# annalam/seqkit

Hardware: AMD Instinct MI355X
Metric: M reads/s demultiplex (150bp, 96 barcodes) at 1/8 GPUs; % HBM roofline (higher is better)
Workload: dtype u8

## Files before the change

### seqkit_amd/csrc/sk_deflate.hip

```cpp
#include <hip/hip_runtime.h>

#include <algorithm>
#include <cstdlib>
#include <cstring>

#include "sk_internal.h"

namespace sk {

typedef uint32_t u32;
typedef unsigned long long u64;
typedef u32 u32x4 __attribute__((ext_vector_type(4)));

constexpr int kDefWaves = 4;
constexpr int kDefHashBits = 12;
constexpr u32 kDefMaxIn = 0xff00u;
constexpr int kNLL = 286, kND = 30;

struct DefLds {
	uint16_t head[1 << kDefHashBits];
	u32 freq[kNLL + kND];
	uint16_t code[kNLL + kND];
	uint8_t len[kNLL + kND + 2];
	u32 nfreq[2 * kNLL];
	uint16_t parent[2 * kNLL];
	uint16_t order[kNLL];
	uint8_t depth[2 * kNLL];
	u32 stage[128];
};

__device__ const uint8_t kPreLen[19] = {4, 5, 5, 5, 4, 4, 4, 4, 4, 4, 4, 4, 4, 4, 4, 4, 5, 5, 5};
__device__ const uint8_t kPreOrderD[19] = {16, 17, 18, 0, 8, 7, 9, 6, 10, 5, 11, 4, 12, 3, 13, 2, 14, 1, 15};

__device__ __forceinline__ void def_fence()
{
	__builtin_amdgcn_fence(__ATOMIC_RELEASE, "wavefront");
	__builtin_amdgcn_wave_barrier();
	__builtin_amdgcn_fence(__ATOMIC_ACQUIRE, "wavefront");
}
__device__ __forceinline__ u32 def_uniform(u32 v) { return (u32)__builtin_amdgcn_readfirstlane((int)v); }
__device__ __forceinline__ u32 def_rev(u32 code, u32 len) { return __builtin_bitreverse32(code) >> (32u - len); }

__device__ __forceinline__ u32 def_load4(const uint8_t *p)
{
	const uintptr_t a = (uintptr_t)p;
	const u32 *q = reinterpret_cast<const u32 *>(a & ~(uintptr_t)3);
	const u32 sh = (u32)(a & 3u);
	const u32 lo = q[0];
	return sh == 0u ? lo : __builtin_amdgcn_alignbyte(q[1], lo, sh);
}

__device__ __forceinline__ void def_len_code(u32 len, u32 &sym, u32 &xb, u32 &xv)
{
	const u32 l = len - 3u;
	if (l < 8u) { sym = 257u + l; xb = 0u; xv = 0u; return; }
	if (len == 258u) { sym = 285u; xb = 0u; xv = 0u; return; }
	const u32 nb = 31u - (u32)__builtin_clz(l);
	sym = 257u + 4u * (nb - 1u) + ((l >> (nb - 2u)) & 3u);
	xb = nb - 2u;
	xv = l & ((1u << xb) - 1u);
}
__device__ __forceinline__ void def_dist_code(u32 dist, u32 &sym, u32 &xb, u32 &xv)
{
	const u32 d = dist - 1u;
	if (d < 4u) { sym = d; xb = 0u; xv = 0u; return; }
	const u32 nb = 31u - (u32)__builtin_clz(d);
	sym = 2u * nb + ((d >> (nb - 1u)) & 1u);
	xb = nb - 1u;
	xv = d & ((1u << xb) - 1u);
}

__device__ __attribute__((noinline)) void def_huffman(int wave, int base, int n, int lane)
{
	extern __shared__ __attribute__((aligned(16))) uint8_t def_smem[];
	DefLds &L = reinterpret_cast<DefLds *>(def_smem)[def_uniform((u32)wave)];
	base = (int)def_uniform((u32)base); n = (int)def_uniform((u32)n);
	u32 *const freq = L.freq + base;
	for (int shift = 0;; shift++) {
		u32 used = 0u;
		for (int s0 = 0; s0 < n; s0 += 64) {
			const int s = s0 + lane;
			used += (u32)__popcll(__ballot(s < n && freq[s] != 0u));
		}
		for (int s = lane; s < n; s += 64) L.len[base + s] = 0;
		if (used == 0u) {
			if (lane == 0) { L.len[base] = 1; L.code[base] = 0; }
			def_fence();
			return;
		}
		if (used == 1u) {
			for (int s = lane; s < n; s += 64) if (freq[s] != 0u) { L.len[base + s] = 1; L.code[base + s] = 0; }
			def_fence();
			return;
		}
		for (int s = lane; s < n; s += 64) {
			const u32 f = freq[s];
			if (f == 0u) continue;
			const u32 fs = max(1u, f >> shift);
			u32 r = 0u;
			for (int t = 0; t < n; t++) {
				const u32 g = freq[t];
				if (g == 0u) continue;
				const u32 gs = max(1u, g >> shift);
				r += (gs < fs || (gs == fs && t < s)) ? 1u : 0u;
			}
			L.order[r] = (uint16_t)s;
			L.nfreq[r] = fs;
		}
		def_fence();
		{
			u32 li = 0u, ii = used, made = used;
			const u32 total = 2u * used - 1u;
			while (made < total) {
				u32 pick[2];
#pragma unroll
				for (int k = 0; k < 2; k++) {
					const bool leaf_ok = li < used, int_ok = ii < made;
					bool take_leaf = leaf_ok;
					if (leaf_ok && int_ok) take_leaf = def_uniform(L.nfreq[li]) <= def_uniform(L.nfreq[ii]);
					pick[k] = take_leaf ? li++ : ii++;
				}
				if (lane == 0) {
					L.nfreq[made] = L.nfreq[pick[0]] + L.nfreq[pick[1]];
					L.parent[pick[0]] = (uint16_t)made;
					L.parent[pick[1]] = (uint16_t)made;
				}
				def_fence();
				made++;
			}
			if (lane == 0) L.depth[total - 1u] = 0;
			def_fence();
			for (int i = (int)total - 2; i >= 0; i--) {
				if (lane == 0) L.depth[i] = (uint8_t)(L.depth[L.parent[i]] + 1);
				def_fence();
			}
		}
		u32 maxd = 0u;
		for (u32 r0 = 0; r0 < used; r0 += 64) {
			const u32 r = r0 + (u32)lane;
			u32 d = r < used ? L.depth[r] : 0u;
			for (int o = 32; o > 0; o >>= 1) d = max(d, (u32)__shfl_xor((int)d, o));
			maxd = max(maxd, d);
		}
		if (maxd > 15u) continue;
		for (u32 r = (u32)lane; r < used; r += 64u) L.len[base + L.order[r]] = L.depth[r];
		def_fence();
		break;
	}
	u32 cnt[16];
#pragma unroll
	for (int l = 0; l < 16; l++) cnt[l] = 0u;
	for (int s0 = 0; s0 < n; s0 += 64) {
		const int s = s0 + lane;
		const u32 ls = s < n ? L.len[base + s] : 0u;
#pragma unroll
		for (int l = 1; l < 16; l++) cnt[l] += (u32)__popcll(__ballot(ls == (u32)l));
	}
	u32 first[16];
	{
		u32 c = 0u;
		first[0] = 0u;
#pragma unroll
		for (int l = 1; l < 16; l++) { c = (c + cnt[l - 1]) << 1; first[l] = c; }
	}
	u32 run[16];
#pragma unroll
	for (int l = 0; l < 16; l++) run[l] = 0u;
	for (int s0 = 0; s0 < n; s0 += 64) {
		const int s = s0 + lane;
		const u32 ls = s < n ? L.len[base + s] : 0u;
#pragma unroll
		for (int l = 1; l < 16; l++) {
			const u64 m = __ballot(ls == (u32)l);
			if (ls == (u32)l) L.code[base + s] = (uint16_t)def_rev(first[l] + run[l] + __builtin_amdgcn_mbcnt_hi((u32)(m >> 32), __builtin_amdgcn_mbcnt_lo((u32)m, 0u)), (u32)l);
			run[l] += (u32)__popcll(m);
		}
	}
	def_fence();
}

struct DefBlock { u64 in_off; u32 in_len, pad; };
static_assert(sizeof(DefBlock) == 16, "== sk_deflate_block");

struct DefOut { u32 *dst; u32 words; u32 carry_bits; };

__global__ __launch_bounds__(kDefWaves * 64) void bgzf_deflate_kernel(const uint8_t *in, const DefBlock *blocks, int64_t n_blocks, uint8_t *out, u32 out_stride,
                                                                      u32 *tokens, u32 *result)
{
	extern __shared__ __attribute__((aligned(16))) uint8_t def_smem[];
	const int lane = threadIdx.x & 63;
	const int wave = __builtin_amdgcn_readfirstlane((int)(threadIdx.x >> 6));
	DefLds &L = reinterpret_cast<DefLds *>(def_smem)[wave];
	for (int64_t bi = (int64_t)blockIdx.x * kDefWaves + wave; bi < n_blocks; bi += (int64_t)gridDim.x * kDefWaves) {
		const u64 in_off = (u64)def_uniform((u32)blocks[bi].in_off) | ((u64)def_uniform((u32)(blocks[bi].in_off >> 32)) << 32);
		const u32 n = def_uniform(blocks[bi].in_len);
		const uint8_t *src = in + in_off;
		u32 *const tok = tokens + (size_t)bi * kDefMaxIn;
		u32 *const dst = reinterpret_cast<u32 *>(out + (size_t)bi * out_stride);
		for (int i = lane; i < (1 << kDefHashBits); i += 64) L.head[i] = 0;
		for (int i = lane; i < kNLL + kND; i += 64) L.freq[i] = 0u;
		def_fence();
		u32 ntok = 0u, skip = 0u;
		for (u32 c0 = 0; c0 < n; c0 += 64u) {
			const u32 p = c0 + (u32)lane;
			const u32 cnt = min(64u, n - c0);
			u32 mlen = 0u, mdist = 0u, v = 0u, h = 0u;
			const bool can = p + 4u <= n;
			if (can) {
				v = def_load4(src + p);
				h = (v * 2654435761u) >> (32 - kDefHashBits);
				const u32 cand1 = L.head[h];
				if (cand1 != 0u) {
					const u32 cand = cand1 - 1u;
					const u32 d = p - cand;
					if (d <= 32768u && def_load4(src + cand) == v) {
						u32 l = 4u;
						const u32 maxl = min(258u, n - p);
						while (l + 4u <= maxl) {
							const u32 x = def_load4(src + cand + l) ^ def_load4(src + p + l);
							if (x != 0u) { l += (u32)__builtin_ctz(x) >> 3; break; }
							l += 4u;
						}
						if (l + 4u > maxl) { while (l < maxl && src[cand + l] == src[p + l]) l++; }
						mlen = l; mdist = d;
					}
				}
			}
			def_fence();
			if (can) L.head[h] = (uint16_t)(p + 1u);
			u64 starts = 0ull;
			u32 q = skip;
			while (q < cnt) {
				const u32 l = (u32)__builtin_amdgcn_readlane((int)mlen, (int)q);
				starts |= 1ull << q;
				q += l >= 3u ? l : 1u;
			}
			skip = q - cnt;
			const bool mine = (starts >> lane) & 1ull;
			const bool is_match = mine && mlen >= 3u;
			if (mine) {
				const u32 rank = __builtin_amdgcn_mbcnt_hi((u32)(starts >> 32), __builtin_amdgcn_mbcnt_lo((u32)starts, 0u));
				u32 t;
				if (is_match) {
					t = 0x80000000u | ((mlen - 3u) << 16) | (mdist - 1u);
					u32 sym, xb, xv;
					def_len_code(mlen, sym, xb, xv);
					atomicAdd(&L.freq[sym], 1u);
					def_dist_code(mdist, sym, xb, xv);
					atomicAdd(&L.freq[kNLL + sym], 1u);
				} else {
					const u32 b = can ? (v & 0xffu) : (u32)src[p];
					t = b;
					atomicAdd(&L.freq[b], 1u);
				}
				tok[ntok + rank] = t;
			}
			ntok += (u32)__popcll(starts);
		}
		if (lane == 0) atomicAdd(&L.freq[256], 1u);
		def_fence();
		def_huffman(wave, 0, kNLL, lane);
		def_huffman(wave, kNLL, kND, lane);
		for (int i = lane; i < 128; i += 64) L.stage[i] = 0u;
		def_fence();
		u32 words = 0u, carry = 0u;
		auto put = [&](u64 bv, u32 nb) {
			u32 off = nb;
#pragma unroll
			for (int o = 1; o < 64; o <<= 1) {
				const u32 t = (u32)__shfl_up((int)off, o);
				if (lane >= o) off += t;
			}
			const u32 total = (u32)__builtin_amdgcn_readlane((int)off, 63);
			const u32 at = carry + off - nb;
			if (nb != 0u) {
				const u32 w = at >> 5, sh = at & 31u;
				const u64 lo = bv << sh;
				atomicOr(&L.stage[w], (u32)lo);
				if (sh + nb > 32u) atomicOr(&L.stage[w + 1u], (u32)(lo >> 32));
				if (sh + nb > 64u) atomicOr(&L.stage[w + 2u], (u32)(bv >> (64u - sh)));
			}
			def_fence();
			const u32 bits = carry + total;
			const u32 full = bits >> 5;
			u32 keep = 0u;
			if ((u32)lane < full) dst[words + (u32)lane] = L.stage[lane];
			if ((u32)lane + 64u < full) dst[words + 64u + (u32)lane] = L.stage[64 + lane];
			keep = def_uniform(L.stage[full]);
			def_fence();
			for (int i = lane; i < 128; i += 64) L.stage[i] = 0u;
			def_fence();
			if (lane == 0) L.stage[0] = keep;
			def_fence();
			words += full;
			carry = bits & 31u;
		};
		{
			u64 bv = 0ull;
			u32 nb = 0u;
			if (lane == 0) { bv = 1ull | (2ull << 1) | (29ull << 3) | (29ull << 8) | (15ull << 13); nb = 17u; }
			else if (lane <= 19) { bv = kPreLen[kPreOrderD[lane - 1]]; nb = 3u; }
			put(bv, nb);
		}
		{
			auto pre_code = [&](u32 s, u32 &cl) -> u32 {
				cl = kPreLen[s];
				u32 before = 0u;
				for (u32 t = 0; t < s; t++) before += kPreLen[t] == cl ? 1u : 0u;
				const u32 c = cl == 4u ? before : (13u << 1) + before;
				return def_rev(c, cl);
			};
			for (int s0 = 0; s0 < kNLL + kND; s0 += 64) {
				const int s = s0 + lane;
				u64 bv = 0ull;
				u32 nb = 0u;
				if (s < kNLL + kND) { u32 cl; bv = pre_code(L.len[s], cl); nb = cl; }
				put(bv, nb);
			}
		}
		for (u32 t0 = 0; t0 < ntok + 1u; t0 += 64u) {
			const u32 ti = t0 + (u32)lane;
			u64 bv = 0ull;
			u32 nb = 0u;
			if (ti < ntok) {
				const u32 t = tok[ti];
				if (t & 0x80000000u) {
					const u32 len = ((t >> 16) & 0xffu) + 3u, dist = (t & 0x7fffu) + 1u;
					u32 sym, xb, xv;
					def_len_code(len, sym, xb, xv);
					bv = L.code[sym]; nb = L.len[sym];
					bv |= (u64)xv << nb; nb += xb;
					def_dist_code(dist, sym, xb, xv);
					bv |= (u64)L.code[kNLL + sym] << nb; nb += L.len[kNLL + sym];
					bv |= (u64)xv << nb; nb += xb;
				} else {
					bv = L.code[t]; nb = L.len[t];
				}
			} else if (ti == ntok) {
				bv = L.code[256]; nb = L.len[256];
			}
			put(bv, nb);
		}
		if (carry != 0u) {
			if (lane == 0) dst[words] = L.stage[0];
			words++;
		}
		if (lane == 0) {
			const u32 nbytes = (words - (carry != 0u ? 1u : 0u)) * 4u + ((carry + 7u) >> 3);
			result[2 * bi] = nbytes;
			result[2 * bi + 1] = ntok;
		}
		def_fence();
	}
}

__device__ __forceinline__ u32 dcrc_mul(u32 a, u32 b)
{
	u32 r = 0u;
	for (int i = 0; i < 32; i++) {
		if (a & 0x80000000u) r ^= b;
		a <<= 1;
		b = (b >> 1) ^ ((b & 1u) ? 0xEDB88320u : 0u);
	}
	return r;
}
__global__ __launch_bounds__(256) void bgzf_crc_out_kernel(const uint8_t *in, const DefBlock *blocks, int64_t n_blocks, u32 *crc_out)
{
	__shared__ u32 tab[4][256];
	__shared__ u32 pw[20];
	{
		u32 c = threadIdx.x;
		for (int k = 0; k < 8; k++) c = (c >> 1) ^ ((c & 1u) ? 0xEDB88320u : 0u);
		tab[0][threadIdx.x] = c;
		__syncthreads();
		u32 t = c;
		for (int k = 1; k < 4; k++) { t = (t >> 8) ^ tab[0][t & 0xffu]; tab[k][threadIdx.x] = t; }
		if (threadIdx.x == 0) {
			u32 p = 0x00800000u;
			for (int k = 0; k < 20; k++) { pw[k] = p; p = dcrc_mul(p, p); }
		}
	}
	__syncthreads();
	const int lane = threadIdx.x & 63, wave = threadIdx.x >> 6;
	for (int64_t bi = (int64_t)blockIdx.x * 4 + wave; bi < n_blocks; bi += (int64_t)gridDim.x * 4) {
		const u32 n = blocks[bi].in_len;
		const uint8_t *p = in + blocks[bi].in_off;
		const u32 mis = (u32)((16u - ((uintptr_t)p & 15u)) & 15u);
		const u32 headn = mis < n ? mis : n;
		const u32 body = n - headn;
		const u32 piece = (((body + 63u) >> 6) + 15u) & ~15u;
		const u32 lo = headn + min(body, piece * (u32)lane), hi = headn + min(body, piece * (u32)lane + piece);
		u32 c = lane == 0 ? 0xFFFFFFFFu : 0u;
		u32 len = hi - lo;
		if (lane == 0) {
			for (u32 i = 0; i < headn; i++) c = tab[0][(c ^ p[i]) & 0xffu] ^ (c >> 8);
			len += headn;
		}
		u32 i = lo;
		for (; i + 16u <= hi; i += 16u) {
			const u32x4 w = *reinterpret_cast<const u32x4 *>(p + i);
#pragma unroll
			for (int k = 0; k < 4; k++) {
				const u32 x = c ^ w[k];
				c = tab[3][x & 0xffu] ^ tab[2][(x >> 8) & 0xffu] ^ tab[1][(x >> 16) & 0xffu] ^ tab[0][x >> 24];
			}
		}
		for (; i < hi; i++) c = tab[0][(c ^ p[i]) & 0xffu] ^ (c >> 8);
		for (int o = 1; o < 64; o <<= 1) {
			const u32 cr = __shfl_down(c, o), lr = __shfl_down(len, o);
			if ((lane & (2 * o - 1)) == 0 && lane + o < 64) {
				u32 sh = 0x80000000u;
				u32 nb = lr;
				for (int k = 0; nb != 0u; k++, nb >>= 1) if (nb & 1u) sh = dcrc_mul(sh, pw[k]);
				c = dcrc_mul(c, sh) ^ cr;
				len += lr;
			}
		}
		if (lane == 0) crc_out[bi] = c ^ 0xFFFFFFFFu;
	}
}

hipError_t launch_bgzf_deflate(const uint8_t *in, const void *blocks, int64_t n_blocks, uint8_t *out, uint32_t out_stride, uint32_t *tokens, uint32_t *result,
                               uint32_t *crc, int n_cu, hipStream_t st)
{
	if (n_blocks <= 0) return hipSuccess;
	static bool attr_set = false;
	const size_t lds = sizeof(DefLds) * kDefWaves;
	if (!attr_set) {
		hipError_t e = hipFuncSetAttribute(reinterpret_cast<const void *>(bgzf_deflate_kernel), hipFuncAttributeMaxDynamicSharedMemorySize, (int)lds);
		if (e != hipSuccess) return e;
		attr_set = true;
	}
	const int per_cu = std::max(1, (int)((160 * 1024) / lds));
	int64_t grid = (n_blocks + kDefWaves - 1) / kDefWaves;
	const int64_t cap = (int64_t)n_cu * per_cu * 4;
	if (grid > cap) grid = cap;
	bgzf_deflate_kernel<<<dim3((unsigned)grid), dim3(kDefWaves * 64), lds, st>>>(in, reinterpret_cast<const DefBlock *>(blocks), n_blocks, out, out_stride, tokens, result);
	hipError_t e = hipGetLastError();
	if (e != hipSuccess) return e;
	int64_t cgrid = (n_blocks + 3) / 4;
	if (cgrid > (int64_t)n_cu * 16) cgrid = (int64_t)n_cu * 16;
	bgzf_crc_out_kernel<<<dim3((unsigned)cgrid), dim3(256), 0, st>>>(in, reinterpret_cast<const DefBlock *>(blocks), n_blocks, crc);
	return hipGetLastError();
}

hipError_t launch_bgzf_crc(const uint8_t *in, const void *blocks, int64_t n_blocks, uint32_t *crc, int n_cu, hipStream_t st)
{
	if (n_blocks <= 0) return hipSuccess;
	int64_t cgrid = (n_blocks + 3) / 4;
	if (cgrid > (int64_t)n_cu * 16) cgrid = (int64_t)n_cu * 16;
	bgzf_crc_out_kernel<<<dim3((unsigned)cgrid), dim3(256), 0, st>>>(in, reinterpret_cast<const DefBlock *>(blocks), n_blocks, crc);
	return hipGetLastError();
}

size_t deflate_tokens_per_block() { return kDefMaxIn; }

}
```

### seqkit_amd/build.py

```python
from __future__ import annotations

import os
import shutil
import subprocess
import sys

ROOT = os.path.dirname(os.path.abspath(__file__))
REPO = os.path.dirname(ROOT)
CSRC = os.path.join(ROOT, "csrc")
LIBDIR = os.path.join(ROOT, "lib")
BINDIR = os.path.join(ROOT, "bin")
LIB_PATH = os.path.join(LIBDIR, "libseqkit_hip.so")

HIP_SOURCES = ["sk_kernels.hip", "sk_census.hip", "sk_inflate.hip", "sk_deflate.hip", "sk_bamtext.hip", "sk_bamwrite.hip", "sk_bamminimize.hip", "sk_bammarkdup.hip", "sk_bamsubsample.hip", "sk_bammerge.hip", "sk_bamcoverage.hip", "sk_bampair.hip", "sk_bamtarget.hip", "sk_capi.hip", "sk_bamfile.cpp", "sk_bamfile_reads.cpp", "sk_bamfile_out.cpp", "sk_bamfile_coverage.cpp", "sk_lut.cpp"]
HIP_DEPS = HIP_SOURCES + ["sk_internal.h", "sk_lut.h", "sk_bamblock.h", "sk_bamfmt.h", "sk_bamfile.h", "sk_passmem.h", "sk_hoststage.h", "sk_tileplan.h", "sk_censusplan.h", os.path.join(REPO, "include", "seqkit_hip.h")]
HIP_FLAGS = ["--offload-arch=gfx950", "-O3", "-std=c++17", "-fPIC", "-shared", "-Wall", "-Wno-unused-function"]


def library_inputs_digest() -> str:
    import hashlib
    h = hashlib.sha256()
    h.update(" ".join(HIP_FLAGS).encode())
    for d in HIP_DEPS:
        p = d if os.path.isabs(d) else os.path.join(CSRC, d)
        with open(p, "rb") as f:
            h.update(os.path.basename(p).encode() + b"\0" + f.read())
    return h.hexdigest()[:16]


def _hipcc() -> str:
    for cand in (os.environ.get("HIPCC"), shutil.which("hipcc"), "/opt/rocm/bin/hipcc"):
        if cand and os.path.exists(cand):
            return cand
    raise RuntimeError("hipcc not found: the gfx950 library cannot be built")


def _stale(target: str, deps: list[str]) -> bool:
    if not os.path.exists(target):
        return True
    t = os.path.getmtime(target)
    for d in deps:
        p = d if os.path.isabs(d) else os.path.join(CSRC, d)
        if os.path.exists(p) and os.path.getmtime(p) > t:
            return True
    return False


def _run(cmd: list[str], cwd: str) -> None:
    r = subprocess.run(cmd, cwd=cwd, stdout=subprocess.PIPE, stderr=subprocess.STDOUT, text=True)
    if r.returncode != 0:
        sys.stderr.write(r.stdout)
        raise RuntimeError("build failed: " + " ".join(cmd))


def build_library(force: bool = False, verbose: bool = False) -> str:
    os.makedirs(LIBDIR, exist_ok=True)
    if force or _stale(LIB_PATH, HIP_DEPS):
        cmd = [_hipcc()] + HIP_FLAGS + ["-o", LIB_PATH] + HIP_SOURCES + ["-ldl", "-lz", "-pthread"]
        if verbose:
            cmd.append("-Rpass-analysis=kernel-resource-usage")
        _run(cmd, CSRC)
    return LIB_PATH


def build_hosts(force: bool = False) -> list[str]:
    os.makedirs(BINDIR, exist_ok=True)
    out = []
    for name, srcs, libs in (("fasta", ["host_common.cpp", "host_inflate.cpp", "fasta_main.cpp", "fasta_text.cpp"], ["-lz", "-ldl"]),
                             ("sam", ["host_common.cpp", "host_inflate.cpp", "sam_main.cpp"], ["-lz", "-ldl"])):
        if not all(os.path.exists(os.path.join(CSRC, s)) for s in srcs):
            continue
        target = os.path.join(BINDIR, name)
        deps = srcs + ["host_common.h", "sam_pairing.h", "sk_bamfmt.h", os.path.join(REPO, "include", "seqkit_hip.h"), LIB_PATH]
        if force or _stale(target, deps):
            cmd = ["g++", "-O2", "-std=c++17", "-Wall", "-Wextra", "-pthread", "-I", os.path.join(REPO, "include"),
                   "-o", target] + srcs + ["-L", LIBDIR, "-lseqkit_hip", "-Wl,-rpath,$ORIGIN/../lib"] + libs
            _run(cmd, CSRC)
        out.append(target)
    return out


def build_all(force: bool = False) -> None:
    build_library(force=force)
    build_hosts(force=force)


if __name__ == "__main__":
    build_all(force="--force" in sys.argv)
    print(LIB_PATH)
```

### seqkit_amd/csrc/sk_bamfile.cpp

```cpp
#include <fcntl.h>
#include <hip/hip_runtime.h>
#include <sys/stat.h>
#include <unistd.h>
#include <zlib.h>

#include <algorithm>
#include <chrono>
#include <cstdio>
#include <cstdlib>
#include <condition_variable>
#include <cstring>
#include <memory>
#include <mutex>
#include <string>
#include <thread>
#include <vector>

#include "sk_bamfile.h"

using namespace bamfile;

namespace {

bool pread_full(int fd, uint8_t *dst, size_t n, uint64_t off)
{
	size_t got = 0;
	while (got < n) {
		const ssize_t r = pread(fd, dst + got, n - got, (off_t)(off + got));
		if (r < 0) { if (errno == EINTR) continue; return false; }
		if (r == 0) return false;
		got += (size_t)r;
	}
	return true;
}

}

struct Mapper {
	OutRange *r = nullptr;
	std::thread th;
	std::mutex m;
	std::condition_variable cv;
	size_t want = 0, have = 0;
	bool stop = false, failed = false;
	void start(OutRange *range)
	{
		r = range; have = r->mapped;
		th = std::thread([this] {
			(void)hipSetDevice(r->device);
			std::unique_lock<std::mutex> lk(m);
			for (;;) {
				cv.wait(lk, [this] { return stop || want > have; });
				if (stop) return;
				const size_t next = have + 1;
				lk.unlock();
				const bool ok = r->ensure(next);
				lk.lock();
				if (!ok) { failed = true; cv.notify_all(); return; }
				have = r->mapped;
				cv.notify_all();
			}
		});
	}
	void ask(size_t bytes) { std::lock_guard<std::mutex> lk(m); if (bytes > want) { want = std::min(bytes, r->reserved); cv.notify_all(); } }
	bool wait_for(size_t bytes) { std::unique_lock<std::mutex> lk(m); if (bytes > want) { want = std::min(bytes, r->reserved); cv.notify_all(); } cv.wait(lk, [&] { return failed || have >= bytes; }); return !failed; }
	~Mapper() { if (th.joinable()) { { std::lock_guard<std::mutex> lk(m); stop = true; cv.notify_all(); } th.join(); } }
};
struct Readers {
	int fd = -1;
	uint8_t *ring = nullptr;
	size_t chunk = 0;
	uint64_t fsize = 0, n_chunks = 0;
	int R = 0;
	std::vector<hipEvent_t> ev;
	std::vector<int64_t> ready, copied;
	std::vector<std::thread> th;
	std::mutex m;
	std::condition_variable cv;
	uint64_t next = 0;
	bool stop = false, failed = false;
	int device = 0;
	void start(int threads)
	{
		ready.assign((size_t)R, -1); copied.assign((size_t)R, -1);
		for (int t = 0; t < threads; t++) th.emplace_back([this] {
			(void)hipSetDevice(device);
			for (;;) {
				uint64_t k;
				{
					std::unique_lock<std::mutex> lk(m);
					if (stop || next >= n_chunks) return;
					k = next++;
					const int s = (int)(k % (uint64_t)R);
					if (k >= (uint64_t)R) {
						cv.wait(lk, [&] { return stop || copied[(size_t)s] == (int64_t)(k - (uint64_t)R); });
						if (stop) return;
					}
				}
				const int s = (int)(k % (uint64_t)R);
				if (k >= (uint64_t)R) (void)hipEventSynchronize(ev[(size_t)s]);
				const uint64_t off = k * chunk;
				const size_t len = (size_t)std::min<uint64_t>(chunk, fsize - off);
				const bool ok = pread_full(fd, ring + (size_t)s * chunk, len, off);
				std::lock_guard<std::mutex> lk(m);
				if (!ok) failed = true;
				ready[(size_t)s] = (int64_t)k;
				cv.notify_all();
			}
		});
	}
	bool wait_ready(uint64_t k)
	{
		std::unique_lock<std::mutex> lk(m);
		const int s = (int)(k % (uint64_t)R);
		cv.wait(lk, [&] { return failed || ready[(size_t)s] == (int64_t)k; });
		return !failed;
	}
	void done_with(uint64_t k)
	{
		std::lock_guard<std::mutex> lk(m);
		copied[(size_t)(k % (uint64_t)R)] = (int64_t)k;
		cv.notify_all();
	}
	~Readers()
	{
		{ std::lock_guard<std::mutex> lk(m); stop = true; cv.notify_all(); }
		for (auto &t : th) t.join();
	}
};

int bamfile::bam_file_front(sk_ctx *c, const char *path, Cleanup &cl, Front &fr, double info[8])
{
	const char *who = fr.who;
	Ranges *both = (Ranges *)sk::ctx_ext(c);
	if (!both) { both = new Ranges; sk::ctx_set_ext(c, both, Ranges::destroy); }
	if (both->reads.busy() || both->rw.busy() || both->pairs.busy()) {
		BF_HIP(hipStreamSynchronize(sk::ctx_stream(c)));
		BF_HIP(hipStreamSynchronize(sk::ctx_stream2(c)));
	}
	both->gen++;
	both->reads.stop();
	both->rw.stop();
	both->pairs.stop();
	cl.fd = open(path, O_RDONLY);
	if (cl.fd < 0) BF_LEAVE(1);
	struct stat sb;
	if (fstat(cl.fd, &sb) != 0 || !S_ISREG(sb.st_mode) || sb.st_size < 28) BF_LEAVE(2);
	const uint64_t fsize = (uint64_t)sb.st_size;
	const double t0 = now_ms();
	hipStream_t st = sk::ctx_stream(c), st2 = sk::ctx_stream2(c);
	cl.wait_for = {st, st2};

	int krc = SK_OK;
	uint64_t out_cap = std::max<uint64_t>(fsize * 6, (uint64_t)256 << 20);
	if (const char *ev = getenv("SK_BAMFILE_OUT_FACTOR")) { const int f = atoi(ev); if (f >= 1 && f <= 1100) out_cap = std::max<uint64_t>(fsize * (uint64_t)f, (uint64_t)1 << 20); }
	uint8_t *d_out = nullptr, *d_comp = nullptr;
	OutRange *range = nullptr, *crange = nullptr;
	if (!getenv("SK_BAMFILE_NO_VMM")) {
		int dev = 0;
		BF_HIP(hipGetDevice(&dev));
		if (both->out.va && both->out.reserved < out_cap + 256) both->out.release();
		if (both->comp.va && both->comp.reserved < fsize + 64) both->comp.release();
		const bool comp_mapped = fsize > ((uint64_t)8 << 30);
		if (!comp_mapped && both->comp.va) both->comp.release();
		if ((both->out.va || both->out.reserve(out_cap + 256, dev)) && (!comp_mapped || both->comp.va || both->comp.reserve(fsize + 64, dev))) {
			range = &both->out;
			crange = comp_mapped ? &both->comp : nullptr;
		}
	}
	Mapper mapper, cmapper;
	if (range) {
		out_cap = range->reserved - 256;
		d_out = range->va;
		if (crange) {
			d_comp = crange->va;
			cmapper.start(crange);
			cmapper.ask((size_t)fsize + 64);
		} else {
			d_comp = (uint8_t *)sk::ctx_keep(c, sk::kKeepComp, fsize + 64, false, &krc);
			if (!d_comp) return krc;
		}
		mapper.start(range);
		mapper.ask(std::min<size_t>((size_t)fsize * 2, range->reserved));
	} else if (sk::ctx_kept_bytes(c, sk::kKeepOut) >= out_cap + 64) {
		out_cap = sk::ctx_kept_bytes(c, sk::kKeepOut) - 64;
		d_out = (uint8_t *)sk::ctx_keep(c, sk::kKeepOut, out_cap + 64, false, &krc);
		d_comp = (uint8_t *)sk::ctx_keep(c, sk::kKeepComp, fsize + 64, false, &krc);
		if (!d_comp) return krc;
	} else {
		d_comp = (uint8_t *)sk::ctx_keep(c, sk::kKeepComp, fsize + 64, false, &krc);
		if (!d_comp) return krc;
		size_t free_b = 0, total_b = 0;
		BF_HIP(hipMemGetInfo(&free_b, &total_b));
		out_cap = std::min<uint64_t>(out_cap, (uint64_t)((free_b + sk::ctx_kept_bytes(c, sk::kKeepOut)) * 0.8));
		d_out = (uint8_t *)sk::ctx_keep(c, sk::kKeepOut, out_cap + 64, false, &krc);
		if (!d_out) BF_LEAVE(3);
	}

	size_t chunk = (size_t)4 << 20;
	if (const char *ev = getenv("SK_BAMFILE_CHUNK_LOG2")) { const int lg = atoi(ev); if (lg >= 12 && lg <= 30) chunk = (size_t)1 << lg; }
	int threads = 8;
	{ const unsigned hc = std::thread::hardware_concurrency(); if (hc >= 1 && hc < 8) threads = (int)hc; }
	if (const char *ev = getenv("SK_BAMFILE_THREADS")) { const int t = atoi(ev); if (t >= 1 && t <= 64) threads = t; }
	const int kBufs = threads + threads / 2 + 1;
	Readers rd;
	rd.fd = cl.fd; rd.chunk = chunk; rd.fsize = fsize; rd.R = kBufs;
	rd.ring = (uint8_t *)sk::ctx_keep(c, sk::kKeepPin, (size_t)kBufs * chunk, true, &krc);
	if (!rd.ring) return krc;
	BF_HIP(hipGetDevice(&rd.device));
	for (int i = 0; i < kBufs; i++) {
		hipEvent_t e;
		BF_HIP(hipEventCreateWithFlags(&e, hipEventDisableTiming));
		cl.events.push_back(e);
		rd.ev.push_back(e);
	}
	hipEvent_t ev_batch;
	BF_HIP(hipEventCreateWithFlags(&ev_batch, hipEventDisableTiming));
	cl.events.push_back(ev_batch);

	const size_t tab_cap = (size_t)(fsize / 8192) + 1024;
	struct BlockTable {
		sk_bgzf_block *p = nullptr;
		size_t n = 0;
		size_t size() const { return n; }
		sk_bgzf_block *data() const { return p; }
		sk_bgzf_block &operator[](size_t i) const { return p[i]; }
	} blocks;
	blocks.p = (sk_bgzf_block *)sk::ctx_keep(c, sk::kKeepTable, tab_cap * sizeof(sk_bgzf_block), true, &krc);
	if (!blocks.p) return krc;
	std::vector<uint64_t> bend;
	bend.reserve(tab_cap);
	sk_bgzf_block *d_blocks = (sk_bgzf_block *)sk::ctx_keep(c, sk::kKeepBlocks, tab_cap * sizeof(sk_bgzf_block), false, &krc);
	if (!d_blocks) return krc;
	uint32_t *d_status = (uint32_t *)sk::ctx_keep(c, sk::kKeepStatus, tab_cap * sizeof(uint32_t), false, &krc);
	if (!d_status) return krc;

	const double t_alloc = now_ms();
	const size_t slots = (size_t)sk::ctx_n_cu(c) * 16;
	size_t min_batch = 2 * slots;
	if (const char *ev = getenv("SK_BAMFILE_BATCH")) { const int v = atoi(ev); if (v >= 1) min_batch = (size_t)v; }
	bool whole_rounds = true, two_streams = true;
	if (const char *ev = getenv("SK_BAMFILE_ROUNDS")) whole_rounds = atoi(ev) != 0;
	if (const char *ev = getenv("SK_BAMFILE_STREAMS")) two_streams = atoi(ev) >= 2;
	hipStream_t st_b = st;
	hipEvent_t ev_b = nullptr;
	if (two_streams) {
		BF_HIP(hipStreamCreateWithFlags(&st_b, hipStreamNonBlocking));
		cl.streams.push_back(st_b);
		BF_HIP(hipEventCreateWithFlags(&ev_b, hipEventDisableTiming));
		cl.events.push_back(ev_b);
	}
	int n_batches = 0;
	uint64_t scan = 0, out_off = 0;
	size_t launched = 0;
	const uint64_t n_chunks = (fsize + chunk - 1) / chunk;
	uint8_t carry[65536 + 64];
	rd.n_chunks = n_chunks;
	rd.start(threads);
	for (uint64_t k = 0; k < n_chunks; k++) {
		const uint64_t c_off = k * chunk;
		const size_t c_len = (size_t)std::min<uint64_t>(chunk, fsize - c_off);
		uint8_t *buf = rd.ring + (size_t)(k % (uint64_t)kBufs) * chunk;
		if (!rd.wait_ready(k)) BF_LEAVE(4);
		if (crange && !cmapper.wait_for((size_t)(c_off + c_len) + 64)) BF_LEAVE(3);
		BF_HIP(hipMemcpyAsync(d_comp + c_off, buf, c_len, hipMemcpyHostToDevice, st2));
		BF_HIP(hipEventRecord(rd.ev[(size_t)(k % (uint64_t)kBufs)], st2));
		const uint64_t have = c_off + c_len;
		auto bytes = [&](uint64_t off, size_t n) -> const uint8_t * {
			if (off >= c_off) return buf + (off - c_off);
			if (n > sizeof carry || !pread_full(cl.fd, carry, n, off)) return nullptr;
			return carry;
		};
		while (scan + 18 <= have) {
			const uint8_t *h = bytes(scan, 18);
			if (!h) BF_LEAVE(5);
			if (h[0] != 31 || h[1] != 139 || h[2] != 8 || !(h[3] & 4)) BF_LEAVE(6);
			const size_t xlen = (size_t)h[10] | ((size_t)h[11] << 8);
			if (scan + 12 + xlen > have) break;
			const uint8_t *x = bytes(scan, 12 + xlen);
			if (!x) BF_LEAVE(7);
			size_t bsize = 0;
			for (size_t o = 12; o + 4 <= 12 + xlen;) {
				const size_t slen = (size_t)x[o + 2] | ((size_t)x[o + 3] << 8);
				if (x[o] == 'B' && x[o + 1] == 'C' && slen == 2 && o + 6 <= 12 + xlen) { bsize = ((size_t)x[o + 4] | ((size_t)x[o + 5] << 8)) + 1; break; }
				o += 4 + slen;
			}
			if (bsize == 0 || bsize < 12 + xlen + 8) BF_LEAVE(8);
			if (scan + bsize > have) break;
			const uint8_t *tr = bytes(scan + bsize - 8, 8);
			if (!tr) BF_LEAVE(9);
			sk_bgzf_block b;
			b.in_off = scan + 12 + xlen;
			b.in_len = (uint32_t)(bsize - 12 - xlen - 8);
			b.crc32 = le32(tr);
			b.out_len = le32(tr + 4);
			b.out_off = out_off;
			b.reserved = 0;
			if (b.out_len > 65536u) BF_LEAVE(10);
			out_off += b.out_len;
			if (out_off > out_cap) BF_LEAVE(11);
			if (blocks.n >= tab_cap) BF_LEAVE(12);
			blocks.p[blocks.n++] = b;
			bend.push_back(out_off);
			scan += bsize;
		}
		size_t n_new = blocks.size() - launched;
		const bool last = k + 1 == n_chunks;
		if (n_new && (n_new >= min_batch || last)) {
			if (!last && whole_rounds && n_new >= slots) n_new -= n_new % slots;
			const size_t first_new = launched;
			if (range) {
				const size_t upto = (size_t)(blocks[first_new + n_new - 1].out_off + blocks[first_new + n_new - 1].out_len) + 128;
				mapper.ask(upto + ((size_t)3 << 29));
				if (!mapper.wait_for(upto)) BF_LEAVE(3);
			}
			hipStream_t sb = (n_batches & 1) ? st_b : st;
			BF_HIP(hipMemcpyAsync(d_blocks + first_new, blocks.data() + first_new, n_new * sizeof(sk_bgzf_block), hipMemcpyHostToDevice, st2));
			BF_HIP(hipEventRecord(ev_batch, st2));
			BF_HIP(hipStreamWaitEvent(sb, ev_batch, 0));
			BF_HIP(sk::launch_bgzf_inflate(d_comp, d_blocks + first_new, (int64_t)n_new, d_out, d_status + first_new, 1, sk::ctx_n_cu(c), sb));
			launched += n_new;
			n_batches++;
		}
		rd.done_with(k);
	}
	if (two_streams) {
		BF_HIP(hipEventRecord(ev_b, st_b));
		BF_HIP(hipStreamWaitEvent(st, ev_b, 0));
	}
	if (scan != fsize) BF_LEAVE(13);
	if (launched != blocks.size()) BF_LEAVE(13);
	const int64_t nb = (int64_t)blocks.size();
	const uint64_t stream_len = out_off;
	const double t_read = now_ms();
	BF_HIP(hipStreamSynchronize(st2));
	std::vector<uint32_t> status((size_t)nb);
	BF_HIP(hipMemcpyAsync(status.data(), d_status, (size_t)nb * 4, hipMemcpyDeviceToHost, st));
	{
		hipEvent_t ev_done;
		BF_HIP(hipEventCreateWithFlags(&ev_done, hipEventBlockingSync | hipEventDisableTiming));
		cl.events.push_back(ev_done);
		BF_HIP(hipEventRecord(ev_done, st));
		BF_HIP(hipEventSynchronize(ev_done));
	}
	const double t_inflated = now_ms();
	uint64_t n_host = 0;
	{
		std::vector<uint8_t> cbuf, obuf;
		for (int64_t i = 0; i < nb; i++) {
			if (status[(size_t)i] == 0) continue;
			const sk_bgzf_block &b = blocks[(size_t)i];
			if (getenv("SK_BAMFILE_TRACE")) fprintf(stderr, "%s: block %lld (in %u bytes at %llu, out %u) has status %#x: zlib\n", who, (long long)i, b.in_len, (unsigned long long)b.in_off, b.out_len, status[(size_t)i]);
			cbuf.resize(b.in_len ? b.in_len : 1);
			obuf.resize(b.out_len ? b.out_len : 1);
			if (b.in_len && !pread_full(cl.fd, cbuf.data(), b.in_len, b.in_off)) BF_LEAVE(14);
			z_stream z;
			memset(&z, 0, sizeof z);
			if (inflateInit2(&z, -15) != Z_OK) BF_LEAVE(15);
			z.next_in = cbuf.data(); z.avail_in = b.in_len;
			z.next_out = obuf.data(); z.avail_out = b.out_len;
			const int zr = inflate(&z, Z_FINISH);
			const bool ok = zr == Z_STREAM_END && z.total_out == b.out_len;
			inflateEnd(&z);
			if (!ok) BF_LEAVE(16);
			if ((uint32_t)crc32(crc32(0L, Z_NULL, 0), obuf.data(), b.out_len) != b.crc32) BF_LEAVE(17);
			if (b.out_len) BF_HIP(hipMemcpy(d_out + b.out_off, obuf.data(), b.out_len, hipMemcpyHostToDevice));
			n_host++;
		}
	}
	bamfmt::RefList refs;
	std::vector<uint8_t> hd;
	for (size_t want = (size_t)std::min<uint64_t>(stream_len, (uint64_t)1 << 20);;) {
		hd.resize(want);
		if (want) BF_HIP(hipMemcpy(hd.data(), d_out, want, hipMemcpyDeviceToHost));
		const bamfmt::RefList::Status rs = refs.parse(hd.data(), want, stream_len);
		if (rs == bamfmt::RefList::kBad) BF_LEAVE(18);
		if (rs == bamfmt::RefList::kOk) break;
		if (want >= stream_len) BF_LEAVE(19);
		want = (size_t)std::min<uint64_t>(stream_len, (uint64_t)want * 4);
	}
	const uint64_t first = refs.end;
	const int32_t n_ref_hdr = refs.n_ref;
	const double t_header = now_ms();
	uint64_t *d_bend = nullptr, *d_entry = nullptr, *d_exit = nullptr;
	uint32_t *d_nrec = nullptr;
	BF_HIP(hipMalloc((void **)&d_bend, (size_t)(nb + 1) * 8)); cl.dev.push_back(d_bend);
	BF_HIP(hipMalloc((void **)&d_entry, (size_t)(nb + 1) * 8)); cl.dev.push_back(d_entry);
	BF_HIP(hipMalloc((void **)&d_exit, (size_t)(nb + 1) * 8)); cl.dev.push_back(d_exit);
	BF_HIP(hipMalloc((void **)&d_nrec, (size_t)(nb + 2) * 4)); cl.dev.push_back(d_nrec);
	BF_HIP(hipMemcpyAsync(d_bend, bend.data(), (size_t)nb * 8, hipMemcpyHostToDevice, st));
	BF_HIP(hipMemsetAsync(d_out + stream_len, 0, 64, st));
	int verified = 0, rounds = 0;
	uint64_t n_records = 0;
	int max_rounds = 64;
	if (const char *ev = getenv("SK_BAMFILE_MAX_ROUNDS")) { const int v = atoi(ev); if (v >= 1) max_rounds = v; }
	if (int r = sk_bam_walk_dev(c, d_out, stream_len, d_bend, nb, first, n_ref_hdr, d_entry, d_exit, d_nrec, max_rounds, &verified, &n_records, &rounds)) return r;
	if (!verified) BF_LEAVE(20);
	fr.nrec.resize((size_t)nb);
	if (nb) BF_HIP(hipMemcpy(fr.nrec.data(), d_nrec, (size_t)nb * 4, hipMemcpyDeviceToHost));
	fr.header.assign(hd.begin(), hd.begin() + (ptrdiff_t)first);
	fr.refs = std::move(refs);
	fr.ready = true;
	fr.d_out = d_out; fr.d_comp = d_comp; fr.stream_len = stream_len; fr.first = first; fr.n_records = n_records; fr.fsize = fsize; fr.n_host = n_host;
	fr.d_bend = d_bend; fr.d_entry = d_entry; fr.nb = nb; fr.rounds = rounds; fr.n_ref = n_ref_hdr;
	fr.t0 = t0; fr.t_alloc = t_alloc; fr.t_read = t_read; fr.t_inflated = t_inflated; fr.t_header = t_header; fr.t_walk = now_ms();
	return SK_OK;
}

void bamfile::file_call_close(const Front &fr, const char *stage, double t_stage, const char *tail, double info[8])
{
	if (getenv("SK_BAMFILE_TRACE"))
		fprintf(stderr, "%s: alloc %.1f ms, read + copy + launches %.1f ms, wait for the inflate %.1f ms, host blocks + header %.1f ms, walk %.1f ms, %s %.1f ms; %lld blocks, %llu by zlib%s\n",
		        fr.who, fr.t_alloc - fr.t0, fr.t_read - fr.t_alloc, fr.t_inflated - fr.t_read, fr.t_header - fr.t_inflated, t_stage - fr.t_header, stage,
		        now_ms() - t_stage, (long long)fr.nb, (unsigned long long)fr.n_host, tail);
	if (!info) return;
	info[0] = (double)fr.fsize; info[1] = (double)fr.stream_len; info[2] = (double)fr.nb; info[3] = (double)fr.n_records;
	info[4] = (double)fr.n_host; info[5] = (double)fr.rounds; info[6] = fr.t_read - fr.t0; info[7] = now_ms() - fr.t_read;
}

int bamfile::block_first_records(sk_ctx *c, const Front &fr, std::vector<uint64_t> &rb)
{
	rb.resize((size_t)fr.nb + 1);
	uint64_t run = 0;
	for (int64_t i = 0; i < fr.nb; i++) { rb[(size_t)i] = run; run += fr.nrec[(size_t)i]; }
	rb[(size_t)fr.nb] = run;
	if (run != fr.n_records)
		return sk::ctx_fail(c, SK_ERR_HIP, "%s: %llu records by the blocks' counts, %llu by the walk", fr.who, (unsigned long long)run, (unsigned long long)fr.n_records);
	return SK_OK;
}

int bamfile::plan_windows(sk_ctx *c, Cleanup &cl, uint64_t window_bytes, const uint64_t *off0, const uint64_t *off1, uint64_t n, uint64_t total0,
                          uint64_t total1, WindowedState &s, std::vector<uint64_t> &w0, std::vector<uint64_t> *w1, uint64_t max[3], bool *room)
{
	*room = true;
	uint64_t W = window_bytes ? window_bytes : (uint64_t)64 << 20;
	W = std::min<uint64_t>(std::max<uint64_t>(W, 256), (uint64_t)1 << 30);
	const int64_t nw = n ? (int64_t)((total0 + total1) / W + 2) : 1;
	s.ws.assign((size_t)nw, n); w0.assign((size_t)nw, total0);
	if (w1) w1->assign((size_t)nw, total1);
	if (n) {
		hipStream_t st = sk::ctx_stream(c);
		uint64_t *d_w = nullptr;
		if (hipMalloc((void **)&d_w, (size_t)nw * (w1 ? 24 : 16)) != hipSuccess) { (void)hipGetLastError(); *room = false; return SK_OK; }
		cl.dev.push_back(d_w);
		BF_HIP(sk::launch_bam_windows(off0, off1, (int64_t)n, W, total0, total1, d_w, d_w + nw, w1 ? d_w + 2 * nw : nullptr, nw, st));
		BF_HIP(hipMemcpyAsync(s.ws.data(), d_w, (size_t)nw * 8, hipMemcpyDeviceToHost, st));
		BF_HIP(hipMemcpyAsync(w0.data(), d_w + nw, (size_t)nw * 8, hipMemcpyDeviceToHost, st));
		if (w1) BF_HIP(hipMemcpyAsync(w1->data(), d_w + 2 * nw, (size_t)nw * 8, hipMemcpyDeviceToHost, st));
		BF_HIP(hipStreamSynchronize(st));
	}
	max[0] = max[1] = max[2] = 0;
	for (size_t w = 0; w + 1 < (size_t)nw; w++) {
		max[0] = std::max(max[0], s.ws[w + 1] - s.ws[w]);
		max[1] = std::max(max[1], w0[w + 1] - w0[w]);
		if (w1) max[2] = std::max(max[2], (*w1)[w + 1] - (*w1)[w]);
	}
	return SK_OK;
}

int bamfile::read_decline(sk_ctx *c, const char *who, const uint32_t *d_decline, uint32_t found)
{
	hipStream_t st = sk::ctx_stream(c);
	uint32_t word = 0;
	hipError_t e = hipMemcpyAsync(&word, d_decline, 4, hipMemcpyDeviceToHost, st);
	if (e == hipSuccess) e = hipStreamSynchronize(st);
	if (e != hipSuccess) { sk::ctx_fail(c, SK_ERR_HIP, "%s: the decline word: %s", who, hipGetErrorString(e)); return -1; }
	word |= found;
	if (word && getenv("SK_BAMFILE_TRACE")) fprintf(stderr, "%s: declined (bits %#x)\n", who, word);
	return (int)word;
}
extern "C" int sk_bam_file_reduce(sk_ctx *c, const char *path, int32_t max_frag, uint64_t counters[3], uint64_t *hist, uint64_t *hist_total,
                                  int *handled, double info[8])
{
	Cleanup cl;
	Front fr;
	if (int r = file_call_open(c, path, "sk_bam_file_reduce", handled, info, cl, fr, [&] {
		    if (max_frag < 0) return sk::ctx_fail(c, SK_ERR_INVALID, "max_frag = %d", max_frag);
		    if (!counters && !hist) return sk::ctx_fail(c, SK_ERR_INVALID, "nothing to do");
		    return (int)SK_OK;
	    }))
		return r;
	if (!fr.ready) return SK_OK;
	hipStream_t st = sk::ctx_stream(c);
	uint64_t *d_red = nullptr;
	const size_t nred = 4 + (size_t)max_frag + 1;
	BF_HIP(hipMalloc((void **)&d_red, nred * 8)); cl.dev.push_back(d_red);
	BF_HIP(hipMemsetAsync(d_red, 0, nred * 8, st));
	if (int r = sk_bam_walk_reduce_dev(c, fr.d_out, fr.stream_len, fr.d_bend, fr.d_entry, fr.nb, max_frag, counters ? 1 : 0, hist ? 1 : 0, d_red)) return r;
	std::vector<uint64_t> red(nred);
	BF_HIP(hipMemcpyAsync(red.data(), d_red, nred * 8, hipMemcpyDeviceToHost, st));
	BF_HIP(hipStreamSynchronize(st));
	if (counters) for (int i = 0; i < 3; i++) counters[i] += red[(size_t)i];
	if (hist) {
		if (hist_total) *hist_total += red[3];
		for (size_t i = 0; i <= (size_t)max_frag; i++) hist[i] += red[4 + i];
	}
	*handled = 1;
	file_call_close(fr, "reduce", fr.t_walk, "", info);
	return SK_OK;
}

extern "C" int sk_bam_file_columns(sk_ctx *c, const char *path, uint32_t want, sk_bam_columns *cols, int *handled, double info[8])
{
	if (!cols) return SK_ERR_INVALID;
	Cleanup cl;
	Front fr;
	if (int r = file_call_open(c, path, "sk_bam_file_columns", handled, info, cl, fr, [&] {
		    memset(cols, 0, sizeof *cols);
		    if (want & ~(uint32_t)SK_COL_ALL) return sk::ctx_fail(c, SK_ERR_INVALID, "want = %#x", want);
		    return (int)SK_OK;
	    }))
		return r;
	if (!fr.ready) return SK_OK;
	hipStream_t st = sk::ctx_stream(c);
	const double t_gather = now_ms();
	const uint64_t n = fr.n_records;
	static const size_t width[8] = {2, 1, 4, 4, 4, 4, 4, 4};
	size_t at[8], total = 0;
	for (int k = 0; k < 8; k++) {
		at[k] = total;
		if (want & (1u << k)) total += up(n * width[k] + 16);
	}
	int krc = SK_OK;
	uint8_t *base = (uint8_t *)sk::ctx_keep(c, sk::kKeepCols, total ? total : 256, false, &krc);
	if (!base) BF_LEAVE(21);
	void *col[8];
	for (int k = 0; k < 8; k++) col[k] = (want & (1u << k)) ? (void *)(base + at[k]) : nullptr;
	std::vector<uint64_t> rb;
	if (int r = block_first_records(c, fr, rb)) return r;
	if (want && fr.nb) {
		uint64_t *d_rb = nullptr;
		BF_HIP(hipMalloc((void **)&d_rb, rb.size() * 8)); cl.dev.push_back(d_rb);
		BF_HIP(hipMemcpyAsync(d_rb, rb.data(), rb.size() * 8, hipMemcpyHostToDevice, st));
		BF_HIP(sk::launch_bam_gather(fr.d_out, fr.stream_len, fr.d_bend, fr.d_entry, d_rb, fr.nb, (uint16_t *)col[0], (uint8_t *)col[1], (int32_t *)col[2],
		                             (int32_t *)col[3], (int32_t *)col[4], (int32_t *)col[5], (int32_t *)col[6], (int32_t *)col[7], st));
	}
	BF_HIP(hipStreamSynchronize(st));
	Ranges *keep = (Ranges *)sk::ctx_ext(c);
	keep->header.swap(fr.header);
	cols->n = (int64_t)n;
	cols->flag = (uint16_t *)col[0]; cols->mapq = (uint8_t *)col[1]; cols->tid = (int32_t *)col[2]; cols->mtid = (int32_t *)col[3];
	cols->pos = (int32_t *)col[4]; cols->mpos = (int32_t *)col[5]; cols->tlen = (int32_t *)col[6]; cols->end_pos = (int32_t *)col[7];
	cols->header = keep->header.data();
	cols->header_len = keep->header.size();
	cols->n_ref = fr.n_ref;
	*handled = 1;
	file_call_close(fr, "gather", t_gather, "", info);
	return SK_OK;
}
```

Measured before the change: 6547.

## Cap per-lane match extension and extend the final match cooperatively across the wave

Each lane's LZ77 match-length scan is now bounded by the remaining lanes in the 64-byte chunk (with a small floor). Lanes already covered by a previous match skip the hash lookup. If the last selected match in a chunk reaches the cap, the whole wave extends it in parallel, each lane comparing 4 bytes, and a ballot finds the first mismatch. This cuts divergent serial compare loops in repetitive data, at the cost of extra readlane/ballot work per chunk and only one cooperative pass of up to 256 bytes.

```diff
diff --git a/seqkit_amd/csrc/sk_deflate.hip b/seqkit_amd/csrc/sk_deflate.hip
--- a/seqkit_amd/csrc/sk_deflate.hip
+++ b/seqkit_amd/csrc/sk_deflate.hip
@@ -15,6 +15,7 @@
 constexpr int kDefWaves = 4;
 constexpr int kDefHashBits = 12;
 constexpr u32 kDefMaxIn = 0xff00u;
+constexpr u32 kDefCapFloor = 16u;
 constexpr int kNLL = 286, kND = 30;
 
 struct DefLds {
@@ -204,25 +205,28 @@
 		for (u32 c0 = 0; c0 < n; c0 += 64u) {
 			const u32 p = c0 + (u32)lane;
 			const u32 cnt = min(64u, n - c0);
-			u32 mlen = 0u, mdist = 0u, v = 0u, h = 0u;
+			u32 mlen = 0u, mdist = 0u, more = 0u, v = 0u, h = 0u;
 			const bool can = p + 4u <= n;
 			if (can) {
 				v = def_load4(src + p);
 				h = (v * 2654435761u) >> (32 - kDefHashBits);
-				const u32 cand1 = L.head[h];
+				const u32 cand1 = (u32)lane >= skip ? L.head[h] : 0u;
 				if (cand1 != 0u) {
 					const u32 cand = cand1 - 1u;
 					const u32 d = p - cand;
 					if (d <= 32768u && def_load4(src + cand) == v) {
 						u32 l = 4u;
 						const u32 maxl = min(258u, n - p);
-						while (l + 4u <= maxl) {
+						const u32 lim = min(maxl, max(kDefCapFloor, cnt - (u32)lane));
+						while (l < lim && l + 4u <= maxl) {
 							const u32 x = def_load4(src + cand + l) ^ def_load4(src + p + l);
 							if (x != 0u) { l += (u32)__builtin_ctz(x) >> 3; break; }
 							l += 4u;
 						}
-						if (l + 4u > maxl) { while (l < maxl && src[cand + l] == src[p + l]) l++; }
+						if (l + 4u > maxl) { while (l < lim && src[cand + l] == src[p + l]) l++; }
+						l = min(l, lim);
 						mlen = l; mdist = d;
+						if (l == lim && lim < maxl) more = maxl;
 					}
 				}
 			}
@@ -234,6 +238,28 @@
 				const u32 l = (u32)__builtin_amdgcn_readlane((int)mlen, (int)q);
 				starts |= 1ull << q;
 				q += l >= 3u ? l : 1u;
+			}
+			if (starts != 0ull) {
+				const u32 sl = 63u - (u32)__builtin_clzll(starts);
+				const u32 maxl = (u32)__builtin_amdgcn_readlane((int)more, (int)sl);
+				if (maxl != 0u) {
+					const u32 l0 = (u32)__builtin_amdgcn_readlane((int)mlen, (int)sl);
+					const uint8_t *const tp = src + c0 + sl, *const sp = tp - (u32)__builtin_amdgcn_readlane((int)mdist, (int)sl);
+					const u32 o = l0 + 4u * (u32)lane;
+					u32 end = ~0u;
+					if (o + 4u <= maxl) {
+						const u32 x = def_load4(sp + o) ^ def_load4(tp + o);
+						if (x != 0u) end = o + ((u32)__builtin_ctz(x) >> 3);
+					} else if (o < maxl) {
+						u32 l = o;
+						while (l < maxl && sp[l] == tp[l]) l++;
+						if (l < maxl) end = l;
+					}
+					const u64 ends = __ballot(end != ~0u);
+					const u32 l1 = ends != 0ull ? (u32)__builtin_amdgcn_readlane((int)end, (int)__builtin_ctzll(ends)) : maxl;
+					if ((u32)lane == sl) mlen = l1;
+					q += l1 - l0;
+				}
 			}
 			skip = q - cnt;
 			const bool mine = (starts >> lane) & 1ull;
```

Result: no change. 6593, median of 3 (+0.7%).

## Ramp inflate batch sizes and launch early when GPU is idle

Applied to the files above, without the earlier changes.

Replaces the fixed minimum batch of two rounds of slots with a feed planner. Batches start at a fraction of one round and double up to a steady size of one round. When event polling shows no batch in flight, the planner launches a small batch early so the GPU is not left waiting while the host parses input. This is meant to cut pipeline startup latency and idle gaps, at the cost of more kernel launches, more event records and queries, and possibly partial rounds that use the CUs less well.

```diff
diff --git a/seqkit_amd/build.py b/seqkit_amd/build.py
--- a/seqkit_amd/build.py
+++ b/seqkit_amd/build.py
@@ -13,7 +13,7 @@
 LIB_PATH = os.path.join(LIBDIR, "libseqkit_hip.so")
 
 HIP_SOURCES = ["sk_kernels.hip", "sk_census.hip", "sk_inflate.hip", "sk_deflate.hip", "sk_bamtext.hip", "sk_bamwrite.hip", "sk_bamminimize.hip", "sk_bammarkdup.hip", "sk_bamsubsample.hip", "sk_bammerge.hip", "sk_bamcoverage.hip", "sk_bampair.hip", "sk_bamtarget.hip", "sk_capi.hip", "sk_bamfile.cpp", "sk_bamfile_reads.cpp", "sk_bamfile_out.cpp", "sk_bamfile_coverage.cpp", "sk_lut.cpp"]
-HIP_DEPS = HIP_SOURCES + ["sk_internal.h", "sk_lut.h", "sk_bamblock.h", "sk_bamfmt.h", "sk_bamfile.h", "sk_passmem.h", "sk_hoststage.h", "sk_tileplan.h", "sk_censusplan.h", os.path.join(REPO, "include", "seqkit_hip.h")]
+HIP_DEPS = HIP_SOURCES + ["sk_internal.h", "sk_lut.h", "sk_bamblock.h", "sk_bamfmt.h", "sk_bamfile.h", "sk_passmem.h", "sk_hoststage.h", "sk_tileplan.h", "sk_censusplan.h", "sk_feedplan.h", os.path.join(REPO, "include", "seqkit_hip.h")]
 HIP_FLAGS = ["--offload-arch=gfx950", "-O3", "-std=c++17", "-fPIC", "-shared", "-Wall", "-Wno-unused-function"]
 
 
diff --git a/seqkit_amd/csrc/sk_bamfile.cpp b/seqkit_amd/csrc/sk_bamfile.cpp
--- a/seqkit_amd/csrc/sk_bamfile.cpp
+++ b/seqkit_amd/csrc/sk_bamfile.cpp
@@ -17,6 +17,7 @@
 #include <vector>
 
 #include "sk_bamfile.h"
+#include "sk_feedplan.h"
 
 using namespace bamfile;
 
@@ -32,6 +33,18 @@
 		got += (size_t)r;
 	}
 	return true;
+}
+
+sk::feedplan::Knobs feed_knobs()
+{
+	sk::feedplan::Knobs k;
+	for (char **e = environ; e && *e; e++) {
+		const char *s = *e;
+		if (strncmp(s, "SK_BAMFILE_", 11) != 0) continue;
+		const char *eq = strchr(s + 11, '=');
+		if (eq) sk::feedplan::set_knob(k, s + 11, (size_t)(eq - (s + 11)), eq + 1);
+	}
+	return k;
 }
 
 }
@@ -236,12 +249,11 @@
 	if (!d_status) return krc;
 
 	const double t_alloc = now_ms();
-	const size_t slots = (size_t)sk::ctx_n_cu(c) * 16;
-	size_t min_batch = 2 * slots;
-	if (const char *ev = getenv("SK_BAMFILE_BATCH")) { const int v = atoi(ev); if (v >= 1) min_batch = (size_t)v; }
-	bool whole_rounds = true, two_streams = true;
-	if (const char *ev = getenv("SK_BAMFILE_ROUNDS")) whole_rounds = atoi(ev) != 0;
-	if (const char *ev = getenv("SK_BAMFILE_STREAMS")) two_streams = atoi(ev) >= 2;
+	const sk::feedplan::Knobs knobs = feed_knobs();
+	sk::feedplan::Facts facts;
+	facts.slots = (size_t)sk::ctx_n_cu(c) * 16;
+	const bool two_streams = knobs.streams >= 2;
+	const bool trace_feed = getenv("SK_BAMFILE_TRACE_FEED") != nullptr;
 	hipStream_t st_b = st;
 	hipEvent_t ev_b = nullptr;
 	if (two_streams) {
@@ -250,6 +262,7 @@
 		BF_HIP(hipEventCreateWithFlags(&ev_b, hipEventDisableTiming));
 		cl.events.push_back(ev_b);
 	}
+	std::vector<hipEvent_t> in_flight, idle_events;
 	int n_batches = 0;
 	uint64_t scan = 0, out_off = 0;
 	size_t launched = 0;
@@ -304,23 +317,45 @@
 			bend.push_back(out_off);
 			scan += bsize;
 		}
-		size_t n_new = blocks.size() - launched;
-		const bool last = k + 1 == n_chunks;
-		if (n_new && (n_new >= min_batch || last)) {
-			if (!last && whole_rounds && n_new >= slots) n_new -= n_new % slots;
+		facts.complete = blocks.size(); facts.launched = launched; facts.batches = n_batches; facts.last = k + 1 == n_chunks;
+		if (facts.complete > launched && !facts.last) {
+			for (size_t i = 0; i < in_flight.size();) {
+				const hipError_t q = hipEventQuery(in_flight[i]);
+				if (q == hipErrorNotReady) { (void)hipGetLastError(); i++; continue; }
+				BF_HIP(q);
+				idle_events.push_back(in_flight[i]);
+				in_flight.erase(in_flight.begin() + (ptrdiff_t)i);
+			}
+		}
+		facts.in_flight = (int)in_flight.size();
+		const sk::feedplan::Feed feed = sk::feedplan::next(knobs, facts);
+		if (const size_t n_new = feed.n) {
 			const size_t first_new = launched;
 			if (range) {
 				const size_t upto = (size_t)(blocks[first_new + n_new - 1].out_off + blocks[first_new + n_new - 1].out_len) + 128;
 				mapper.ask(upto + ((size_t)3 << 29));
 				if (!mapper.wait_for(upto)) BF_LEAVE(3);
 			}
-			hipStream_t sb = (n_batches & 1) ? st_b : st;
+			hipStream_t sb = feed.stream ? st_b : st;
 			BF_HIP(hipMemcpyAsync(d_blocks + first_new, blocks.data() + first_new, n_new * sizeof(sk_bgzf_block), hipMemcpyHostToDevice, st2));
 			BF_HIP(hipEventRecord(ev_batch, st2));
 			BF_HIP(hipStreamWaitEvent(sb, ev_batch, 0));
 			BF_HIP(sk::launch_bgzf_inflate(d_comp, d_blocks + first_new, (int64_t)n_new, d_out, d_status + first_new, 1, sk::ctx_n_cu(c), sb));
+			if (!facts.last) {
+				hipEvent_t e;
+				if (idle_events.empty()) {
+					BF_HIP(hipEventCreateWithFlags(&e, hipEventDisableTiming));
+					cl.events.push_back(e);
+				} else {
+					e = idle_events.back();
+					idle_events.pop_back();
+				}
+				BF_HIP(hipEventRecord(e, sb));
+				in_flight.push_back(e);
+			}
 			launched += n_new;
 			n_batches++;
+			if (trace_feed) fprintf(stderr, "%s: batch %d: %zu blocks from %zu on stream %d after %.2f ms, %d in flight\n", who, n_batches, n_new, first_new, feed.stream, now_ms() - t0, facts.in_flight);
 		}
 		rd.done_with(k);
 	}
diff --git a/seqkit_amd/csrc/sk_feedplan.h b/seqkit_amd/csrc/sk_feedplan.h
--- /dev/null
+++ b/seqkit_amd/csrc/sk_feedplan.h
@@ -0,0 +1,79 @@
+#pragma once
+#include <stddef.h>
+#include <stdlib.h>
+#include <string.h>
+
+namespace sk {
+namespace feedplan {
+
+constexpr int kFirstDiv = 4;
+constexpr int kSteadyRounds = 1;
+
+struct Knobs {
+	size_t batch = 0;
+	bool whole_rounds = true;
+	int streams = 2;
+	int first_div = kFirstDiv;
+	int steady_rounds = kSteadyRounds;
+};
+
+inline void set_knob(Knobs &k, const char *name, size_t len, const char *value)
+{
+	auto is = [&](const char *n) { return strlen(n) == len && memcmp(n, name, len) == 0; };
+	const int v = atoi(value);
+	if (is("BATCH")) { if (v >= 1) k.batch = (size_t)v; }
+	else if (is("ROUNDS")) k.whole_rounds = v != 0;
+	else if (is("STREAMS")) k.streams = v >= 2 ? 2 : 1;
+	else if (is("FIRST_DIV")) { if (v >= 1 && v <= 64) k.first_div = v; }
+	else if (is("STEADY")) { if (v >= 1 && v <= 8) k.steady_rounds = v; }
+}
+
+struct Facts {
+	size_t slots = 0;
+	size_t complete = 0;
+	size_t launched = 0;
+	int batches = 0;
+	int in_flight = 0;
+	bool last = false;
+};
+
+struct Feed {
+	size_t n;
+	int stream;
+};
+
+inline size_t first_step(const Knobs &k, size_t slots) { const size_t f = slots / (size_t)k.first_div; return f ? f : 1; }
+inline size_t steady_size(const Knobs &k, size_t slots) { return (size_t)k.steady_rounds * slots; }
+inline size_t least_batch(const Knobs &k, size_t slots, int batches)
+{
+	if (k.batch) return k.batch;
+	const size_t steady = steady_size(k, slots);
+	size_t need = first_step(k, slots);
+	for (int b = 0; b < batches && need < steady; b++) need *= 2;
+	return need < steady ? need : steady;
+}
+inline int ramp_steps(const Knobs &k, size_t slots)
+{
+	if (k.batch) return 0;
+	int b = 0;
+	while (least_batch(k, slots, b) < steady_size(k, slots)) b++;
+	return b;
+}
+
+inline Feed next(const Knobs &k, const Facts &f)
+{
+	Feed out{0, k.streams >= 2 ? f.batches & 1 : 0};
+	size_t n = f.complete - f.launched;
+	if (n == 0) return out;
+	if (!f.last) {
+		size_t need = least_batch(k, f.slots, f.batches);
+		if (!k.batch && f.in_flight == 0 && need > first_step(k, f.slots)) need = first_step(k, f.slots);
+		if (n < need) return out;
+		if (k.whole_rounds && n >= f.slots) n -= n % f.slots;
+	}
+	out.n = n;
+	return out;
+}
+
+}
+}
```

Result: slower. 6747 before, 6606 after (-2.1%).
